# DarlingHang/st-nerf

Hardware: NVIDIA H100
Metric: rays/sec (higher is better)
Workload: dtype f32 via fp16x3 split products (wgmma), f32 accumulate

## Files before the change

### st-nerf_b200/csrc/mlp_tc.cu

```cuda
#include <cuda_fp16.h>
#include <string.h>
#include <type_traits>
#include <vector>
#include "mlp_tc.cuh"
#include "resample.cuh"

namespace stnerf {

namespace {

constexpr int TILE_M = 128;
constexpr int ABLOCK = 16384;
constexpr int STAGE_BYTES = 16384;
constexpr int NTHREADS = 384;
constexpr int MATH_WG0 = 1, N_MATH_WARPS = 8;
constexpr int MAX_STAGE = 8;
constexpr int BAR_WFULL = 0, BAR_WEMPTY = 8, BAR_RAWFULL = 16, BAR_RAWEMPTY = 18;
constexpr int MISC_ROWS = 256;
constexpr int MISC_PART = MISC_ROWS + 128 * 24;
constexpr int MISC_CDF = MISC_PART + 2048;
constexpr int MISC_TOTAL = MISC_CDF + 512;

__device__ __forceinline__ uint32_t smem_u32(const void* p) { return (uint32_t)__cvta_generic_to_shared(p); }

__device__ __forceinline__ void mbar_init(uint32_t bar, uint32_t count) {
  asm volatile("mbarrier.init.shared::cta.b64 [%0], %1;" ::"r"(bar), "r"(count) : "memory");
}
__device__ __forceinline__ void mbar_arrive(uint32_t bar) {
  asm volatile("mbarrier.arrive.shared::cta.b64 _, [%0];" ::"r"(bar) : "memory");
}
__device__ __forceinline__ void mbar_arrive_if(uint32_t bar, bool pred) {
  asm volatile("{\n\t.reg .pred p;\n\tsetp.ne.b32 p, %1, 0;\n\t@p mbarrier.arrive.shared::cta.b64 _, [%0];\n\t}" ::"r"(bar), "r"((uint32_t)pred)
               : "memory");
}
__device__ __forceinline__ void mbar_expect_tx(uint32_t bar, uint32_t bytes) {
  asm volatile("mbarrier.arrive.expect_tx.shared::cta.b64 _, [%0], %1;" ::"r"(bar), "r"(bytes) : "memory");
}
__device__ __forceinline__ void mbar_wait(uint32_t bar, uint32_t parity) {
  asm volatile(
      "{\n\t.reg .pred p;\n\t.reg .u32 c;\n\t"
      "mov.u32 c, 0;\n"
      "WAIT_%=:\n\t"
      "mbarrier.try_wait.parity.shared::cta.b64 p, [%0], %1;\n\t"
      "@p bra.uni DONE_%=;\n\t"
      "add.u32 c, c, 1;\n\t"
      "setp.gt.u32 p, c, 67108864;\n\t"
      "@p trap;\n\t"
      "bra.uni WAIT_%=;\n"
      "DONE_%=:\n\t}" ::"r"(bar), "r"(parity)
      : "memory");
}
__device__ __forceinline__ void bulk_g2s(uint32_t dst, const void* src, uint32_t bytes, uint32_t bar) {
  asm volatile("cp.async.bulk.shared::cluster.global.mbarrier::complete_tx::bytes [%0], [%1], %2, [%3];" ::"r"(dst),
               "l"(src), "r"(bytes), "r"(bar)
               : "memory");
}
__device__ __forceinline__ void fence_proxy_async() { asm volatile("fence.proxy.async.shared::cta;" ::: "memory"); }
__device__ __forceinline__ void wg_bar_sync(int wg) { asm volatile("bar.sync %0, 128;" ::"r"(1 + wg) : "memory"); }

__device__ __forceinline__ void load_stage_elect(uint32_t dst, const void* src, uint32_t bytes, uint32_t bar) {
  asm volatile(
      "{\n\t.reg .pred pe;\n\t"
      "elect.sync _|pe, 0xffffffff;\n\t"
      "@pe mbarrier.arrive.expect_tx.shared::cta.b64 _, [%3], %2;\n\t"
      "@pe cp.async.bulk.shared::cluster.global.mbarrier::complete_tx::bytes [%0], [%1], %2, [%3];\n\t}" ::"r"(dst),
      "l"(src), "r"(bytes), "r"(bar)
      : "memory");
}

__device__ __forceinline__ uint64_t desc_sw128(uint32_t saddr) {
  return (uint64_t)((saddr >> 4) & 0x3FFF) | ((uint64_t)1 << 16) | ((uint64_t)(1024 >> 4) << 32) | ((uint64_t)1 << 62);
}
__device__ __forceinline__ uint64_t desc_sw64(uint32_t saddr) {
  return (uint64_t)((saddr >> 4) & 0x3FFF) | ((uint64_t)1 << 16) | ((uint64_t)(512 >> 4) << 32) | ((uint64_t)2 << 62);
}
__device__ __forceinline__ void wgmma_fence() { asm volatile("wgmma.fence.sync.aligned;" ::: "memory"); }
__device__ __forceinline__ void wgmma_commit() { asm volatile("wgmma.commit_group.sync.aligned;" ::: "memory"); }
template <int N>
__device__ __forceinline__ void wgmma_wait() { asm volatile("wgmma.wait_group.sync.aligned %0;" ::"n"(N) : "memory"); }
template <int R>
__device__ __forceinline__ void acc_fence(float (&d)[128]) {
#pragma unroll
  for (int i = 0; i < R; ++i) asm volatile("" : "+f"(d[i])::"memory");
}

__device__ __forceinline__ void wgmma_n256(float (&d)[128], uint64_t da, uint64_t db) {
  asm volatile(
      "{\n\t.reg .pred p;\n\tsetp.ne.b32 p, %130, 0;\n\t"
      "wgmma.mma_async.sync.aligned.m64n256k16.f32.f16.f16 "
      "{%0, %1, %2, %3, %4, %5, %6, %7, %8, %9, %10, %11, %12, %13, %14, %15, "
      "%16, %17, %18, %19, %20, %21, %22, %23, %24, %25, %26, %27, %28, %29, %30, %31, "
      "%32, %33, %34, %35, %36, %37, %38, %39, %40, %41, %42, %43, %44, %45, %46, %47, "
      "%48, %49, %50, %51, %52, %53, %54, %55, %56, %57, %58, %59, %60, %61, %62, %63, "
      "%64, %65, %66, %67, %68, %69, %70, %71, %72, %73, %74, %75, %76, %77, %78, %79, "
      "%80, %81, %82, %83, %84, %85, %86, %87, %88, %89, %90, %91, %92, %93, %94, %95, "
      "%96, %97, %98, %99, %100, %101, %102, %103, %104, %105, %106, %107, %108, %109, %110, %111, "
      "%112, %113, %114, %115, %116, %117, %118, %119, %120, %121, %122, %123, %124, %125, %126, %127}, "
      "%128, %129, p, 1, 1, 0, 0;\n\t}"
      : "+f"(d[0]), "+f"(d[1]), "+f"(d[2]), "+f"(d[3]), "+f"(d[4]), "+f"(d[5]), "+f"(d[6]), "+f"(d[7]),
        "+f"(d[8]), "+f"(d[9]), "+f"(d[10]), "+f"(d[11]), "+f"(d[12]), "+f"(d[13]), "+f"(d[14]), "+f"(d[15]),
        "+f"(d[16]), "+f"(d[17]), "+f"(d[18]), "+f"(d[19]), "+f"(d[20]), "+f"(d[21]), "+f"(d[22]), "+f"(d[23]),
        "+f"(d[24]), "+f"(d[25]), "+f"(d[26]), "+f"(d[27]), "+f"(d[28]), "+f"(d[29]), "+f"(d[30]), "+f"(d[31]),
        "+f"(d[32]), "+f"(d[33]), "+f"(d[34]), "+f"(d[35]), "+f"(d[36]), "+f"(d[37]), "+f"(d[38]), "+f"(d[39]),
        "+f"(d[40]), "+f"(d[41]), "+f"(d[42]), "+f"(d[43]), "+f"(d[44]), "+f"(d[45]), "+f"(d[46]), "+f"(d[47]),
        "+f"(d[48]), "+f"(d[49]), "+f"(d[50]), "+f"(d[51]), "+f"(d[52]), "+f"(d[53]), "+f"(d[54]), "+f"(d[55]),
        "+f"(d[56]), "+f"(d[57]), "+f"(d[58]), "+f"(d[59]), "+f"(d[60]), "+f"(d[61]), "+f"(d[62]), "+f"(d[63]),
        "+f"(d[64]), "+f"(d[65]), "+f"(d[66]), "+f"(d[67]), "+f"(d[68]), "+f"(d[69]), "+f"(d[70]), "+f"(d[71]),
        "+f"(d[72]), "+f"(d[73]), "+f"(d[74]), "+f"(d[75]), "+f"(d[76]), "+f"(d[77]), "+f"(d[78]), "+f"(d[79]),
        "+f"(d[80]), "+f"(d[81]), "+f"(d[82]), "+f"(d[83]), "+f"(d[84]), "+f"(d[85]), "+f"(d[86]), "+f"(d[87]),
        "+f"(d[88]), "+f"(d[89]), "+f"(d[90]), "+f"(d[91]), "+f"(d[92]), "+f"(d[93]), "+f"(d[94]), "+f"(d[95]),
        "+f"(d[96]), "+f"(d[97]), "+f"(d[98]), "+f"(d[99]), "+f"(d[100]), "+f"(d[101]), "+f"(d[102]), "+f"(d[103]),
        "+f"(d[104]), "+f"(d[105]), "+f"(d[106]), "+f"(d[107]), "+f"(d[108]), "+f"(d[109]), "+f"(d[110]), "+f"(d[111]),
        "+f"(d[112]), "+f"(d[113]), "+f"(d[114]), "+f"(d[115]), "+f"(d[116]), "+f"(d[117]), "+f"(d[118]), "+f"(d[119]),
        "+f"(d[120]), "+f"(d[121]), "+f"(d[122]), "+f"(d[123]), "+f"(d[124]), "+f"(d[125]), "+f"(d[126]), "+f"(d[127])
      : "l"(da), "l"(db), "r"(1));
}
__device__ __forceinline__ void wgmma_n128(float (&d)[128], uint64_t da, uint64_t db) {
  asm volatile(
      "{\n\t.reg .pred p;\n\tsetp.ne.b32 p, %66, 0;\n\t"
      "wgmma.mma_async.sync.aligned.m64n128k16.f32.f16.f16 "
      "{%0, %1, %2, %3, %4, %5, %6, %7, %8, %9, %10, %11, %12, %13, %14, %15, "
      "%16, %17, %18, %19, %20, %21, %22, %23, %24, %25, %26, %27, %28, %29, %30, %31, "
      "%32, %33, %34, %35, %36, %37, %38, %39, %40, %41, %42, %43, %44, %45, %46, %47, "
      "%48, %49, %50, %51, %52, %53, %54, %55, %56, %57, %58, %59, %60, %61, %62, %63}, "
      "%64, %65, p, 1, 1, 0, 0;\n\t}"
      : "+f"(d[0]), "+f"(d[1]), "+f"(d[2]), "+f"(d[3]), "+f"(d[4]), "+f"(d[5]), "+f"(d[6]), "+f"(d[7]),
        "+f"(d[8]), "+f"(d[9]), "+f"(d[10]), "+f"(d[11]), "+f"(d[12]), "+f"(d[13]), "+f"(d[14]), "+f"(d[15]),
        "+f"(d[16]), "+f"(d[17]), "+f"(d[18]), "+f"(d[19]), "+f"(d[20]), "+f"(d[21]), "+f"(d[22]), "+f"(d[23]),
        "+f"(d[24]), "+f"(d[25]), "+f"(d[26]), "+f"(d[27]), "+f"(d[28]), "+f"(d[29]), "+f"(d[30]), "+f"(d[31]),
        "+f"(d[32]), "+f"(d[33]), "+f"(d[34]), "+f"(d[35]), "+f"(d[36]), "+f"(d[37]), "+f"(d[38]), "+f"(d[39]),
        "+f"(d[40]), "+f"(d[41]), "+f"(d[42]), "+f"(d[43]), "+f"(d[44]), "+f"(d[45]), "+f"(d[46]), "+f"(d[47]),
        "+f"(d[48]), "+f"(d[49]), "+f"(d[50]), "+f"(d[51]), "+f"(d[52]), "+f"(d[53]), "+f"(d[54]), "+f"(d[55]),
        "+f"(d[56]), "+f"(d[57]), "+f"(d[58]), "+f"(d[59]), "+f"(d[60]), "+f"(d[61]), "+f"(d[62]), "+f"(d[63])
      : "l"(da), "l"(db), "r"(1));
}

template <int N>
__device__ __forceinline__ void wgmma_k16(float (&d)[128], uint64_t da, uint64_t db) {
  if (N == 256) wgmma_n256(d, da, db);
  else wgmma_n128(d, da, db);
}

__device__ __forceinline__ uint32_t pack_f16x2(float a, float b) {
  uint32_t r;
  asm("cvt.rn.satfinite.f16x2.f32 %0, %1, %2;" : "=r"(r) : "f"(b), "f"(a));
  return r;
}
__device__ __forceinline__ float2 unpack_f16x2(uint32_t p) {
  return __half22float2(*reinterpret_cast<const __half2*>(&p));
}

__host__ __device__ inline uint32_t sw128_offset(int row, int col) {
  return (uint32_t)((row >> 3) * 1024 + (row & 7) * 128 + ((((col >> 3) ^ (row & 7)) & 7) << 4) + ((col & 7) << 1));
}
__host__ __device__ inline uint32_t sw64_offset(int row, int col) {
  return (uint32_t)((row >> 3) * 512 + (row & 7) * 64 + ((((col >> 3) ^ ((row >> 1) & 3)) & 3) << 4) + ((col & 7) << 1));
}

enum { NET_SPACE = 0, NET_MOTION = 1 };

template <int NET> struct Sched;
template <> struct Sched<NET_SPACE> {
  static constexpr int N_LAYERS = 8;
  static constexpr int act_base = 0, enc_base = 8 * ABLOCK;
  static constexpr int LO_STRIDE = 4 * ABLOCK;
  static constexpr int ENC_LO_STRIDE = ABLOCK;
  static constexpr int n_stage = 3, stage_bytes = STAGE_BYTES;
  static constexpr int ring_base = 10 * ABLOCK, misc_base = ring_base + n_stage * stage_bytes, smem_total = misc_base + MISC_TOTAL;
  static_assert(smem_total <= 232448, "shared memory budget (227 KB per CTA)");
  __host__ __device__ static constexpr int n_out(int l) { return l == 7 ? 128 : 256; }
  __host__ __device__ static constexpr int act_chunks(int l) { return l == 0 ? 0 : 4; }
  __host__ __device__ static constexpr int enc_chunks(int l) { return (l == 0 || l == 4) ? 1 : 0; }
  __host__ __device__ static constexpr bool enc_first(int l) { return l == 4; }
};
template <> struct Sched<NET_MOTION> {
  static constexpr int N_LAYERS = 5;
  static constexpr int act_base = 0, enc_base = 0;
  static constexpr int LO_STRIDE = 2 * ABLOCK;
  static constexpr int ENC_LO_STRIDE = 2 * ABLOCK;
  static constexpr int n_stage = 8, stage_bytes = 8192;
  static constexpr int ring_base = 4 * ABLOCK, misc_base = ring_base + n_stage * stage_bytes, smem_total = misc_base + MISC_TOTAL;
  __host__ __device__ static constexpr int n_out(int) { return 128; }
  __host__ __device__ static constexpr int act_chunks(int l) { return l == 0 ? 0 : 2; }
  __host__ __device__ static constexpr int enc_chunks(int l) { return l == 0 ? 2 : 0; }
  __host__ __device__ static constexpr bool enc_first(int) { return false; }
};
static_assert(Sched<NET_SPACE>::n_stage <= MAX_STAGE && Sched<NET_MOTION>::n_stage <= MAX_STAGE, "barrier slots");

enum { A_HI = 0, A_LO = 1, A_HI_LO = 2 };
template <int A>
struct WStep {
  static constexpr int a = A;
  uint32_t offset;
  uint32_t sub;
};
template <int NET>
struct WSched {
  using S = Sched<NET>;
  __host__ __device__ static constexpr int n_chunks(int l) { return S::act_chunks(l) + S::enc_chunks(l); }
  __host__ __device__ static constexpr uint32_t stage_bytes(int l) { return (uint32_t)S::n_out(l) * 64; }
  __host__ __device__ static constexpr size_t layer_bytes(int l) { return (size_t)n_chunks(l) * 2  * 2  * stage_bytes(l); }
  __host__ __device__ static constexpr int chunk_at(int l, int c) {
    return S::enc_first(l) ? (c == 0 ? S::act_chunks(l) : c - 1) : c;
  }
  static constexpr bool enc_first_valid() {
    for (int l = 0; l < S::N_LAYERS; ++l)
      if (S::enc_first(l) && (S::act_chunks(l) == 0 || S::enc_chunks(l) == 0)) return false;
    return true;
  }
  static_assert(enc_first_valid(), "enc_first(l) needs activation chunks and an encoding chunk to reorder");
  template <bool LOFIRST, class C, class F>
  __device__ __forceinline__ static void for_each_step(int l, bool split, C&& chunk, F&& f) {
    const int nact = S::act_chunks(l), nch = nact + S::enc_chunks(l);
    const uint32_t bytes = stage_bytes(l);
    auto at = [&](const auto& a, int c, uint32_t sub, uint32_t lo_stage, auto op) {
      f(a, WStep<decltype(op)::value>{(2 * (2 * (uint32_t)c + sub) + lo_stage) * bytes, sub});
    };
    using HI = std::integral_constant<int, A_HI>;
    using LO = std::integral_constant<int, A_LO>;
    using HI_LO = std::integral_constant<int, A_HI_LO>;
    if (!LOFIRST || !split) {
      for (int c = 0; c < nch; ++c) {
        const auto a = chunk(chunk_at(l, c));
        for (uint32_t sub = 0; sub < 2; ++sub) {
          if (split) { at(a, c, sub, 1u, HI()); at(a, c, sub, 0u, HI_LO()); }
          else at(a, c, sub, 0u, HI());
        }
      }
    } else {
      for (int c = 0; c < nch; ++c) {
        const auto a = chunk(chunk_at(l, c));
        for (uint32_t sub = 0; sub < 2; ++sub) { at(a, c, sub, 1u, HI()); at(a, c, sub, 0u, LO()); }
      }
      for (int c = 0; c < nch; ++c) {
        const auto a = chunk(chunk_at(l, c));
        for (uint32_t sub = 0; sub < 2; ++sub) at(a, c, sub, 0u, HI());
      }
    }
  }
};

template <int NET>
__host__ __device__ constexpr size_t stream_bytes_per_tile() {
  size_t n = 0;
  for (int l = 0; l < Sched<NET>::N_LAYERS; ++l) n += WSched<NET>::layer_bytes(l);
  return n;
}

struct TcParams {
  FuseCoarse fuse;
  PointSrc src;
  const uint8_t* wstream;
  const float* aux;
  const float* cbuf;
  int exact;
  int single_last;
  int lo_first;
  float* raw;
  float* rgb_out;
  float* sigma_out;
  float* xyz_out;
  float* flow_out;
  const int* lerp_flag;
  int lerp_force;
};

constexpr int AUX_BIAS = 0, AUX_WSIG = 8 * 256, AUX_BSIG = AUX_WSIG + 256, AUX_WOUT = AUX_BSIG + 4,
              AUX_BOUT = AUX_WOUT + 3 * 128, AUX_FLOATS = AUX_BOUT + 4;


struct Pt { float x, y, z, tm; int out_index; int cidx; };

__device__ __forceinline__ Pt fetch_pt(const PointSrc& s, long long p, long long n_points) {
  Pt q;
  q.x = q.y = q.z = q.tm = 0.f;
  q.out_index = -1;
  q.cidx = 0;
  if (p >= n_points) return q;
  if (s.mode == SRC_EXPLICIT) {
    const float* pp = s.pos + p * s.pos_stride;
    q.x = pp[0]; q.y = pp[1]; q.z = pp[2];
    if (s.times) q.tm = s.times[p * s.time_stride];
    q.out_index = (int)p;
    q.cidx = (int)p;
    return q;
  }
  const long long slot = p / s.S;
  const int k = (int)(p - slot * s.S);
  const long long ray = s.hit ? (long long)s.hit[slot] : slot;
  const float* rp = s.rays + ray * s.ray_stride;
  q.tm = rp[6 + s.layer];
  q.out_index = (int)(ray * s.S + k);
  q.cidx = (int)slot;
  if (s.mode == SRC_XYZ) {
    q.x = s.pos[3 * p]; q.y = s.pos[3 * p + 1]; q.z = s.pos[3 * p + 2];
    return q;
  }
  if (s.mode == SRC_XYZ_MAP) {
    const int m = s.src_map[ray * s.S + k];
    const float* pp = (m < s.n_first) ? s.pos + 3 * (slot * s.n_first + m) : s.pos2 + 3 * (slot * (s.S - s.n_first) + (m - s.n_first));
    q.x = pp[0]; q.y = pp[1]; q.z = pp[2];
    return q;
  }
  const float tt = s.t[ray * s.S + k];
  float v[3] = {__fadd_rn(__fmul_rn(tt, rp[3]), rp[0]), __fadd_rn(__fmul_rn(tt, rp[4]), rp[1]),
                __fadd_rn(__fmul_rn(tt, rp[5]), rp[2])};
#pragma unroll
  for (int a = 0; a < 3; ++a) {
    if (s.shift_on) v[a] = __fsub_rn(v[a], s.shift[a]);
    if (s.scale_on) v[a] = __fadd_rn(__fdiv_rn(__fsub_rn(v[a], s.pivot[a]), s.scale), s.pivot[a]);
  }
  q.x = v[0]; q.y = v[1]; q.z = v[2];
  return q;
}

struct SinCos3 { float s0, s1, s2, c0, c1, c2; };
struct SinCos4 { float s0, s1, s2, s3, c0, c1, c2, c3; };
__device__ __noinline__ SinCos3 sincos_full3(float x0, float x1, float x2) {
  SinCos3 r;
  sincosf(x0, &r.s0, &r.c0); sincosf(x1, &r.s1, &r.c1); sincosf(x2, &r.s2, &r.c2);
  return r;
}
__device__ __noinline__ SinCos4 sincos_full4(float x0, float x1, float x2, float x3) {
  SinCos4 r;
  sincosf(x0, &r.s0, &r.c0); sincosf(x1, &r.s1, &r.c1); sincosf(x2, &r.s2, &r.c2); sincosf(x3, &r.s3, &r.c3);
  return r;
}

template <int NV>
__device__ __forceinline__ void store_row_split(uint8_t* hi_blk, int lo_stride, int row, int col0, const float (&v)[NV],
                                                bool exact) {
#pragma unroll
  for (int g = 0; g < NV / 8; ++g) {
    uint32_t hp[4], lp[4];
#pragma unroll
    for (int e = 0; e < 4; ++e) {
      const float a = v[g * 8 + 2 * e], b = v[g * 8 + 2 * e + 1];
      hp[e] = pack_f16x2(a, b);
      const float2 hf = unpack_f16x2(hp[e]);
      lp[e] = pack_f16x2(a - hf.x, b - hf.y);
    }
    const uint32_t off = sw128_offset(row, col0 + g * 8);
    *reinterpret_cast<uint4*>(hi_blk + off) = make_uint4(hp[0], hp[1], hp[2], hp[3]);
    if (exact) *reinterpret_cast<uint4*>(hi_blk + lo_stride + off) = make_uint4(lp[0], lp[1], lp[2], lp[3]);
  }
}

template <int half, int piece>
__device__ __forceinline__ void encode_space_piece(uint8_t* smem, const Pt& pt, int row, bool exact, float (&carry)[2]) {
  using S = Sched<NET_SPACE>;
  uint8_t* enc = smem + S::enc_base;
  const float xs[3] = {pt.x, pt.y, pt.z};
  float v[16];
  auto trig = [&](int f, float* dst) {
    const float fr = (float)(1 << f);
    const SinCos3 q = sincos_full3(xs[0] * fr, xs[1] * fr, xs[2] * fr);
    dst[0] = q.s0; dst[1] = q.s1; dst[2] = q.s2; dst[3] = q.c0; dst[4] = q.c1; dst[5] = q.c2;
  };
  if (piece == 0) {
    float t3[6];
    trig(5 * half + 0, v); trig(5 * half + 1, v + 6); trig(5 * half + 2, t3);
    v[12] = t3[0]; v[13] = t3[1]; v[14] = t3[2]; v[15] = t3[3];
    carry[0] = t3[4]; carry[1] = t3[5];
  } else {
    v[0] = carry[0]; v[1] = carry[1];
    trig(5 * half + 3, v + 2); trig(5 * half + 4, v + 8);
    v[14] = half == 0 ? xs[0] : xs[2];
    v[15] = half == 0 ? xs[1] : 0.f;
  }
  store_row_split<16>(enc, S::ENC_LO_STRIDE, row, half * 32 + piece * 16, v, exact);
}

template <int half, int piece>
__device__ __forceinline__ void encode_motion_piece(uint8_t* smem, const Pt& pt, int row, bool exact, bool lerp) {
  using S = Sched<NET_MOTION>;
  uint8_t* enc = smem + S::enc_base + half * ABLOCK;
  const float lo_t = floorf(pt.tm), wgt = pt.tm - lo_t, omw = 1.0f - wgt;
  const float in4[4] = {pt.x, pt.y, pt.z, pt.tm};
  auto trig = [&](int f, float* dst) {
    const float fr = (float)(1 << f);
    if (!lerp) {
      const SinCos4 q = sincos_full4(in4[0] * fr, in4[1] * fr, in4[2] * fr, in4[3] * fr);
      dst[0] = q.s0; dst[1] = q.s1; dst[2] = q.s2; dst[3] = q.s3; dst[4] = q.c0; dst[5] = q.c1; dst[6] = q.c2; dst[7] = q.c3;
    } else {
      const SinCos4 q = sincos_full4(in4[0] * fr, in4[1] * fr, in4[2] * fr, lo_t * fr);
      const SinCos3 q1 = sincos_full3((lo_t + 1.0f) * fr, 0.f, 0.f);
      const float s0[4] = {q.s0, q.s1, q.s2, q.s3}, c0[4] = {q.c0, q.c1, q.c2, q.c3};
      const float s1[4] = {q.s0, q.s1, q.s2, q1.s0}, c1[4] = {q.c0, q.c1, q.c2, q1.c0};
#pragma unroll
      for (int d = 0; d < 4; ++d) {
        dst[d] = __fadd_rn(__fmul_rn(omw, s0[d]), __fmul_rn(wgt, s1[d]));
        dst[4 + d] = __fadd_rn(__fmul_rn(omw, c0[d]), __fmul_rn(wgt, c1[d]));
      }
    }
  };
  float v[16];
  trig(5 * half + 2 * piece, v);
  if (piece < 2) {
    trig(5 * half + 2 * piece + 1, v + 8);
  } else {
#pragma unroll
    for (int d = 0; d < 4; ++d) {
      float a = 0.f;
      if (half == 0) {
        a = in4[d];
        if (lerp) {
          const float lo = d < 3 ? in4[d] : lo_t, hi = d < 3 ? in4[d] : lo_t + 1.0f;
          a = __fadd_rn(__fmul_rn(omw, lo), __fmul_rn(wgt, hi));
        }
      }
      v[8 + d] = a; v[12 + d] = 0.f;
    }
  }
  store_row_split<16>(enc, S::ENC_LO_STRIDE, row, piece * 16, v, exact);
}

template <int NET, int piece>
__device__ __forceinline__ void encode_piece(uint8_t* smem, const Pt& pt, int row, int half, bool exact, bool lerp,
                                             float (&carry)[2]) {
  if (NET == NET_SPACE) {
    if (half == 0) encode_space_piece<0, piece < 2 ? piece : 1>(smem, pt, row, exact, carry);
    else encode_space_piece<1, piece < 2 ? piece : 1>(smem, pt, row, exact, carry);
  } else {
    if (half == 0) encode_motion_piece<0, piece>(smem, pt, row, exact, lerp);
    else encode_motion_piece<1, piece>(smem, pt, row, exact, lerp);
  }
}

template <int NZ>
__device__ __noinline__ void fused_composite_loop(const TcParams& P, const float* rows, float* cdf, uint32_t bar_full, uint32_t bar_empty,
                                                  long long n_tiles, int j, int lane) {
  const FuseCoarse& F = P.fuse;
  const PointSrc& src = P.src;
  const long long n_slots = src.count ? (long long)(*src.count) : src.n_slots;
  const int n1 = 64, n2 = F.n2;
  uint32_t n = 0;
  for (long long tile = blockIdx.x; tile < n_tiles; tile += gridDim.x, ++n) {
    mbar_wait(bar_full, n & 1);
    const long long slot = tile * 2 + j;
    if (slot < n_slots) {
      const long long ray = src.hit ? (long long)src.hit[slot] : slot;
      const float* tp = src.t + ray * n1;
      const float4* rp = reinterpret_cast<const float4*>(rows) + j * 64;
      float t[2], sg[2];
#pragma unroll
      for (int s = 0; s < 2; ++s) {
        const int k = s * 32 + lane;
        const float tk = __ldg(tp + k);
        float v = rp[k].w;
        if (F.is_bkgd) {
          if (tk < F.near_plane) v = 0.0f;
        } else {
          if (tk < 0.0f) v = 0.0f;
          if (F.apply_thr && v < F.thr) v = 0.0f;
        }
        t[s] = tk;
        sg[s] = v;
      }
      const float* up = F.u ? F.u + ray * n2 : nullptr;
      const uint64_t seed = F.seed;
      const uint32_t stream = 64u + (uint32_t)F.layer;
      const unsigned long long gid = F.idmap(F.ray_base + ray);
      rs::LayerOut lo;
      rs::composite_resample_ray<2, NZ>(
          t, sg, n1, n2, F.boarder,
          [rp, lane](int s) {
            const float4 v = rp[s * 32 + lane];
            return make_float3(__fdiv_rn(1.0f, __fadd_rn(1.0f, expf(-v.x))), __fdiv_rn(1.0f, __fadd_rn(1.0f, expf(-v.y))),
                               __fdiv_rn(1.0f, __fadd_rn(1.0f, expf(-v.z))));
          },
          [up, seed, stream, gid](int jj) { return up ? up[jj] : philox_uniform(seed, stream, gid, (uint32_t)jj); },
          cdf, F.t_fine + ray * (n1 + n2), lane, lo, F.z_new ? F.z_new + ray * n2 : nullptr,
          F.z_new ? F.src_map + ray * (n1 + n2) : nullptr);
      if (F.img && lane < 5) {
        const long long rg = F.ray_base + ray;
        const float v = lane == 0 ? lo.pix[0] : lane == 1 ? lo.pix[1] : lane == 2 ? lo.pix[2] : lane == 3 ? lo.pix[3] : lo.pix[4];
        if (F.pixels) F.img[rg * 5 + lane] = v;
        else if (lane < 3) F.img[rg * 3 + lane] = v;
        else F.img[(long long)lane * F.n_total + rg] = v;
      }
    }
    __syncwarp();
    if (lane == 0) mbar_arrive(bar_empty);
  }
}

template <int NET, int N, bool LOFIRST>
__device__ __forceinline__ void mma_layer(float (&acc)[128], int l, bool sp, uint32_t sbase, uint32_t a_row, uint32_t bars,
                                          uint32_t& cnt, int lane) {
  using S = Sched<NET>;
  using W = WSched<NET>;
  constexpr uint32_t NST = S::n_stage;
#pragma unroll
  for (int i = 0; i < N / 2; ++i) acc[i] = 0.f;
  acc_fence<N / 2>(acc);
  wgmma_fence();
  const int nact = S::act_chunks(l);
  int pend = -1;
  auto release = [&](int s) {
    __syncwarp();
    mbar_arrive_if(bars + 8u * (uint32_t)(BAR_WEMPTY + s), lane == 0);
  };
  auto a_block = [&](int ch) {
    uint32_t hi, lo;
    if (ch < nact) {
      hi = sbase + S::act_base + ch * ABLOCK + a_row;
      lo = hi + S::LO_STRIDE;
    } else {
      hi = sbase + S::enc_base + (ch - nact) * ABLOCK + a_row;
      lo = hi + S::ENC_LO_STRIDE;
    }
    return make_uint2(hi, lo);
  };
  W::template for_each_step<LOFIRST>(l, sp, a_block, [&](const uint2& a, auto st) {
    const uint32_t hi = a.x + 64u * st.sub, lo = a.y + 64u * st.sub;
    const uint32_t a0 = decltype(st)::a == A_LO ? lo : hi;
    const uint32_t s = cnt % NST, n = cnt / NST;
    mbar_wait(bars + 8u * (BAR_WFULL + s), n & 1);
    const uint32_t w = sbase + S::ring_base + s * S::stage_bytes;
#pragma unroll
    for (int ks = 0; ks < 2; ++ks) wgmma_k16<N>(acc, desc_sw128(a0 + ks * 32), desc_sw64(w + ks * 32));
    if constexpr (decltype(st)::a == A_HI_LO) {
#pragma unroll
      for (int ks = 0; ks < 2; ++ks) wgmma_k16<N>(acc, desc_sw128(lo + ks * 32), desc_sw64(w + ks * 32));
    }
    wgmma_commit();
    wgmma_wait<1>();
    if (pend >= 0) release(pend);
    pend = (int)s;
    ++cnt;
  });
  wgmma_wait<0>();
  acc_fence<N / 2>(acc);
  release(pend);
}

template <int NET, int N, bool SIGMA>
__device__ __forceinline__ void epi_hidden(const float (&acc)[128], const float* __restrict__ bias, const float* __restrict__ wsig,
                                           uint8_t* smem, int r0, int cq, bool lo_too, float& sig0, float& sig1) {
  using S = Sched<NET>;
#pragma unroll
  for (int j = 0; j < N / 8; ++j) {
    const int col = 8 * j + cq;
    const float2 b = __ldg(reinterpret_cast<const float2*>(bias + col));
    const float v00 = fmaxf(acc[4 * j] + b.x, 0.f), v01 = fmaxf(acc[4 * j + 1] + b.y, 0.f);
    const float v10 = fmaxf(acc[4 * j + 2] + b.x, 0.f), v11 = fmaxf(acc[4 * j + 3] + b.y, 0.f);
    if (SIGMA) {
      const float2 w = __ldg(reinterpret_cast<const float2*>(wsig + col));
      sig0 = fmaf(v00, w.x, sig0); sig0 = fmaf(v01, w.y, sig0);
      sig1 = fmaf(v10, w.x, sig1); sig1 = fmaf(v11, w.y, sig1);
    }
    uint8_t* blk = smem + S::act_base + (col >> 6) * ABLOCK;
    const uint32_t o0 = sw128_offset(r0, col & 63), o1 = sw128_offset(r0 + 8, col & 63);
    const uint32_t h0 = pack_f16x2(v00, v01), h1 = pack_f16x2(v10, v11);
    *reinterpret_cast<uint32_t*>(blk + o0) = h0;
    *reinterpret_cast<uint32_t*>(blk + o1) = h1;
    if (lo_too) {
      const float2 f0 = unpack_f16x2(h0), f1 = unpack_f16x2(h1);
      *reinterpret_cast<uint32_t*>(blk + S::LO_STRIDE + o0) = pack_f16x2(v00 - f0.x, v01 - f0.y);
      *reinterpret_cast<uint32_t*>(blk + S::LO_STRIDE + o1) = pack_f16x2(v10 - f1.x, v11 - f1.y);
    }
  }
}

__device__ __forceinline__ float quad_sum(float v) {
  v += __shfl_xor_sync(0xffffffffu, v, 1);
  v += __shfl_xor_sync(0xffffffffu, v, 2);
  return v;
}

template <int NET, bool LOFIRST>
__global__ void __launch_bounds__(NTHREADS, 1) mlp_tc_kernel(const __grid_constant__ TcParams P) {
  using S = Sched<NET>;
  extern __shared__ __align__(1024) uint8_t smem[];
  const uint32_t sbase = smem_u32(smem);
  if ((sbase & 1023u) != 0) {
    if (threadIdx.x == 0) printf("stnerf mlp_tc: dynamic shared memory base %u is not 1024-byte aligned\n", sbase);
    __trap();
  }
  const uint32_t bars = sbase + S::misc_base;
  auto BAR = [bars](int i) { return bars + 8u * (uint32_t)i; };
  Pt* s_rows = reinterpret_cast<Pt*>(smem + S::misc_base + MISC_ROWS);
  float* s_part = reinterpret_cast<float*>(smem + S::misc_base + MISC_PART);

  const int tid = threadIdx.x, lane = tid & 31;
  const int warp = __shfl_sync(0xffffffffu, tid >> 5, 0);
  const int wgi = __shfl_sync(0xffffffffu, tid >> 7, 0);
  const bool exact = P.exact != 0;
  const bool single_last = P.single_last != 0;
  auto split = [&](int l) { return exact && !(single_last && l == S::N_LAYERS - 1); };
  const long long n_points = src_num_points(P.src);
  const long long n_tiles = (n_points + TILE_M - 1) / TILE_M;
  constexpr uint32_t NST = S::n_stage;
  if (tid == 0) {
    for (int i = 0; i < MAX_STAGE; ++i) { mbar_init(BAR(BAR_WFULL + i), 1); mbar_init(BAR(BAR_WEMPTY + i), N_MATH_WARPS); }
    for (int j = 0; j < 2; ++j) {
      mbar_init(BAR(BAR_RAWFULL + j), 4);
      mbar_init(BAR(BAR_RAWEMPTY + j), 1);
    }
    asm volatile("fence.mbarrier_init.release.cluster;" ::: "memory");
  }
  __syncthreads();

  if (warp == 0) {
    using W = WSched<NET>;
    uint32_t cnt = 0;
    for (long long tile = blockIdx.x; tile < n_tiles; tile += gridDim.x) {
      const uint8_t* layer = P.wstream;
      for (int l = 0; l < S::N_LAYERS; ++l) {
        W::template for_each_step<LOFIRST>(l, split(l), [](int) { return 0; }, [&](int, auto st) {
          const uint32_t s = cnt % NST, n = cnt / NST;
          mbar_wait(BAR(BAR_WEMPTY + s), (n & 1) ^ 1);
          load_stage_elect(sbase + S::ring_base + s * S::stage_bytes, layer + st.offset, W::stage_bytes(l), BAR(BAR_WFULL + s));
          ++cnt;
        });
        layer += W::layer_bytes(l);
      }
    }
  } else if (NET == NET_SPACE && (warp == 2 || warp == 3)) {
    if (P.fuse.on) {
      const int j = warp - 2;
      float* cdf = reinterpret_cast<float*>(smem + S::misc_base + MISC_CDF) + j * 64;
      if (P.fuse.n2 <= 128)
        fused_composite_loop<4>(P, s_part, cdf, BAR(BAR_RAWFULL + j), BAR(BAR_RAWEMPTY + j), n_tiles, j, lane);
      else
        fused_composite_loop<8>(P, s_part, cdf, BAR(BAR_RAWFULL + j), BAR(BAR_RAWEMPTY + j), n_tiles, j, lane);
    }
  } else if (wgi >= MATH_WG0) {
    const int wg = wgi - MATH_WG0;
    const int wt = tid & 127;
    const int erow = wg * 64 + (wt & 63), ehalf = wt >> 6;
    const int r0 = wg * 64 + (wt >> 5) * 16 + (lane >> 2);
    const int cq = 2 * (lane & 3);
    const uint32_t a_row = (uint32_t)wg * 8u * 1024u;
    const float* bias_all = P.aux + AUX_BIAS;
    const bool lerp = (NET == NET_MOTION) && (P.lerp_force >= 0 ? (P.lerp_force != 0) : (P.lerp_flag && *P.lerp_flag != 0));
    const bool fused = (NET == NET_SPACE) && P.fuse.on;
    uint32_t cnt = 0, tile_no = 0;
    float acc[128];
    for (long long tile = blockIdx.x; tile < n_tiles; tile += gridDim.x, ++tile_no) {
      wg_bar_sync(wg);
      const Pt cur = fetch_pt(P.src, tile * TILE_M + erow, n_points);
      if (ehalf == 0) s_rows[erow] = cur;
      float carry[2] = {0.f, 0.f};
      if (NET == NET_MOTION) {
        uint8_t* enc = smem + S::enc_base + ehalf * ABLOCK;
        for (int c = (ehalf == 0 ? 48 : 40); c < 64; c += 8) {
          const uint32_t off = sw128_offset(erow, c);
          *reinterpret_cast<uint4*>(enc + off) = make_uint4(0, 0, 0, 0);
          *reinterpret_cast<uint4*>(enc + S::ENC_LO_STRIDE + off) = make_uint4(0, 0, 0, 0);
        }
      }
      encode_piece<NET, 0>(smem, cur, erow, ehalf, exact, lerp, carry);
      encode_piece<NET, 1>(smem, cur, erow, ehalf, exact, lerp, carry);
      if (NET == NET_MOTION) encode_piece<NET, 2>(smem, cur, erow, ehalf, exact, lerp, carry);
      float sig0 = 0.f, sig1 = 0.f;
      for (int l = 0; l < S::N_LAYERS; ++l) {
        fence_proxy_async();
        wg_bar_sync(wg);
        const bool last = (l == S::N_LAYERS - 1);
        if (!last) {
          mma_layer<NET, (NET == NET_SPACE ? 256 : 128), LOFIRST>(acc, l, split(l), sbase, a_row, bars, cnt, lane);
          if (NET == NET_SPACE && l == 6)
            epi_hidden<NET, 256, true>(acc, bias_all + l * 256, P.aux + AUX_WSIG, smem, r0, cq, split(l + 1), sig0, sig1);
          else
            epi_hidden<NET, (NET == NET_SPACE ? 256 : 128), false>(acc, bias_all + l * 256, nullptr, smem, r0, cq, split(l + 1), sig0, sig1);
          continue;
        }
        mma_layer<NET, 128, LOFIRST>(acc, l, split(l), sbase, a_row, bars, cnt, lane);
        const Pt p0 = s_rows[r0], p1 = s_rows[r0 + 8];
        const float* b0 = (NET == NET_SPACE) ? (P.cbuf + (size_t)p0.cidx * 128) : bias_all + l * 256;
        const float* b1 = (NET == NET_SPACE) ? (P.cbuf + (size_t)p1.cidx * 128) : bias_all + l * 256;
        float d0[3] = {0.f, 0.f, 0.f}, d1[3] = {0.f, 0.f, 0.f};
#pragma unroll
        for (int j = 0; j < 16; ++j) {
          const int col = 8 * j + cq;
          const float2 ba = __ldg(reinterpret_cast<const float2*>(b0 + col));
          const float2 bb = __ldg(reinterpret_cast<const float2*>(b1 + col));
          const float v00 = fmaxf(acc[4 * j] + ba.x, 0.f), v01 = fmaxf(acc[4 * j + 1] + ba.y, 0.f);
          const float v10 = fmaxf(acc[4 * j + 2] + bb.x, 0.f), v11 = fmaxf(acc[4 * j + 3] + bb.y, 0.f);
#pragma unroll
          for (int o = 0; o < 3; ++o) {
            const float2 w = __ldg(reinterpret_cast<const float2*>(P.aux + AUX_WOUT + o * 128 + col));
            d0[o] = fmaf(v00, w.x, d0[o]); d0[o] = fmaf(v01, w.y, d0[o]);
            d1[o] = fmaf(v10, w.x, d1[o]); d1[o] = fmaf(v11, w.y, d1[o]);
          }
        }
#pragma unroll
        for (int o = 0; o < 3; ++o) { d0[o] = quad_sum(d0[o]) + P.aux[AUX_BOUT + o]; d1[o] = quad_sum(d1[o]) + P.aux[AUX_BOUT + o]; }
        if (NET == NET_SPACE) { sig0 = quad_sum(sig0) + P.aux[AUX_BSIG]; sig1 = quad_sum(sig1) + P.aux[AUX_BSIG]; }
        if (fused) {
          if (tile_no > 0) mbar_wait(BAR(BAR_RAWEMPTY + wg), (tile_no - 1) & 1);
          if ((lane & 3) == 0) {
            reinterpret_cast<float4*>(s_part)[r0] = make_float4(d0[0], d0[1], d0[2], sig0);
            reinterpret_cast<float4*>(s_part)[r0 + 8] = make_float4(d1[0], d1[1], d1[2], sig1);
          }
          __syncwarp();
          if (lane == 0) mbar_arrive(BAR(BAR_RAWFULL + wg));
        }
        if ((lane & 3) == 0) {
#pragma unroll
          for (int h = 0; h < 2; ++h) {
            const Pt& p = h ? p1 : p0;
            const float* o = h ? d1 : d0;
            const float sg = h ? sig1 : sig0;
            if (p.out_index < 0) continue;
            const int oi = p.out_index;
            if (NET == NET_SPACE) {
              if (P.raw) reinterpret_cast<float4*>(P.raw)[oi] = make_float4(o[0], o[1], o[2], sg);
              if (P.rgb_out) { P.rgb_out[3 * (size_t)oi] = o[0]; P.rgb_out[3 * (size_t)oi + 1] = o[1]; P.rgb_out[3 * (size_t)oi + 2] = o[2]; }
              if (P.sigma_out) P.sigma_out[oi] = sg;
            } else {
              const long long pidx = tile * TILE_M + r0 + 8 * h;
              if (P.flow_out) { P.flow_out[3 * pidx] = o[0]; P.flow_out[3 * pidx + 1] = o[1]; P.flow_out[3 * pidx + 2] = o[2]; }
              if (P.xyz_out) {
                P.xyz_out[3 * pidx] = __fadd_rn(p.x, o[0]);
                P.xyz_out[3 * pidx + 1] = __fadd_rn(p.y, o[1]);
                P.xyz_out[3 * pidx + 2] = __fadd_rn(p.z, o[2]);
              }
            }
          }
        }
      }
    }
  }
}

constexpr int HB_SLOTS = 8;
__global__ void __launch_bounds__(128) head_bias_kernel(PointSrc src, const float* __restrict__ w_tail ,
                                                        const float* __restrict__ b1, int use_time,
                                                        float* __restrict__ cbuf) {
  __shared__ float s_enc[HB_SLOTS][48];
  const long long n_slots = src.count ? (long long)(*src.count) : src.n_slots;
  const int nk = PE_DIR + (use_time ? PE_TIME : 0);
  const int tid = threadIdx.x;
  float w[48];
#pragma unroll
  for (int k = 0; k < 48; ++k) w[k] = (k < nk) ? __ldg(w_tail + k * 128 + tid) : 0.f;
  const float bias = __ldg(b1 + tid);
  for (long long s0 = (long long)blockIdx.x * HB_SLOTS; s0 < n_slots; s0 += (long long)gridDim.x * HB_SLOTS) {
    __syncthreads();
    for (int e = tid; e < HB_SLOTS * 48; e += 128) {
      const int sl = e / 48, j = e - sl * 48;
      const long long slot = s0 + sl;
      float v = 0.f;
      if (slot < n_slots && j < nk) {
        float d[3], tm;
        if (src.mode == SRC_EXPLICIT) {
          d[0] = src.dirs[3 * slot]; d[1] = src.dirs[3 * slot + 1]; d[2] = src.dirs[3 * slot + 2];
          tm = src.times ? src.times[slot * src.time_stride] : 0.f;
        } else {
          const long long ray = src.hit ? (long long)src.hit[slot] : slot;
          const float* rp = src.rays + ray * src.ray_stride;
          d[0] = rp[3]; d[1] = rp[4]; d[2] = rp[5];
          tm = rp[6 + src.layer];
        }
        if (j < PE_DIR) {
          if (j < 3) v = d[j];
          else {
            const int r = j - 3, f = r / 6, m = r - 6 * f;
            const float a = d[m % 3] * (float)(1 << f);
            v = (m < 3) ? sinf(a) : cosf(a);
          }
        } else {
          const int r = j - PE_DIR;
          if (r == 0) v = tm;
          else {
            const int f = (r - 1) >> 1;
            const float a = tm * (float)(1 << f);
            v = ((r - 1) & 1) ? cosf(a) : sinf(a);
          }
        }
        v = fmaxf(v, 0.f);
      }
      s_enc[sl][j] = v;
    }
    __syncthreads();
#pragma unroll
    for (int sl = 0; sl < HB_SLOTS; ++sl) {
      const long long slot = s0 + sl;
      if (slot >= n_slots) break;
      float acc = bias;
#pragma unroll
      for (int k = 0; k < 48; ++k) acc = fmaf(w[k], s_enc[sl][k], acc);
      cbuf[slot * 128 + tid] = acc;
    }
  }
}

__global__ void __launch_bounds__(256, 1) wgmma_selftest_kernel(const float* __restrict__ A, const uint8_t* __restrict__ Bstages,
                                                               float* __restrict__ D, int reps) {
  extern __shared__ __align__(1024) uint8_t smem[];
  const uint32_t sbase = smem_u32(smem);
  const uint32_t bar = sbase + ABLOCK + 2 * STAGE_BYTES;
  const int tid = threadIdx.x, wg = tid >> 7, wt = tid & 127, lane = tid & 31;
  if ((sbase & 1023u) != 0) __trap();
  if (tid == 0) {
    mbar_init(bar, 1);
    asm volatile("fence.mbarrier_init.release.cluster;" ::: "memory");
  }
  if (tid < 128) {
    for (int c0 = 0; c0 < 64; c0 += 32) {
      float v[32];
      for (int i = 0; i < 32; ++i) v[i] = A[tid * 64 + c0 + i];
      store_row_split<32>(smem, 0, tid, c0, v, false);
    }
  }
  fence_proxy_async();
  __syncthreads();
  if (tid == 0) {
    mbar_expect_tx(bar, 2 * STAGE_BYTES);
    bulk_g2s(sbase + ABLOCK, Bstages, 2 * STAGE_BYTES, bar);
  }
  mbar_wait(bar, 0);
  float acc[128];
#pragma unroll
  for (int i = 0; i < 128; ++i) acc[i] = 0.f;
  acc_fence<128>(acc);
  wgmma_fence();
  for (int rep = 0; rep < reps; ++rep) {
#pragma unroll
    for (int sub = 0; sub < 2; ++sub)
#pragma unroll
      for (int ks = 0; ks < 2; ++ks)
        wgmma_n256(acc, desc_sw128(sbase + (uint32_t)wg * 8192u + sub * 64 + ks * 32),
                   desc_sw64(sbase + ABLOCK + sub * STAGE_BYTES + ks * 32));
    wgmma_commit();
    wgmma_wait<0>();
  }
  acc_fence<128>(acc);
  const int r0 = wg * 64 + (wt >> 5) * 16 + (lane >> 2), cq = 2 * (lane & 3);
#pragma unroll
  for (int j = 0; j < 32; ++j) {
    const int col = 8 * j + cq;
    D[r0 * 256 + col] = acc[4 * j];
    D[r0 * 256 + col + 1] = acc[4 * j + 1];
    D[(r0 + 8) * 256 + col] = acc[4 * j + 2];
    D[(r0 + 8) * 256 + col + 1] = acc[4 * j + 3];
  }
}

struct LayerSpec { const float* W; int N, K_total; std::vector<std::vector<int>> chunks; };

std::vector<int> iota_chunk(int k0, int kend) {
  std::vector<int> c(64, -1);
  for (int i = 0; i < 64 && k0 + i < kend; ++i) c[i] = k0 + i;
  return c;
}
std::vector<int> enc_perm_space(int base) {
  std::vector<int> c(64, -1);
  for (int h = 0; h < 2; ++h) {
    for (int ff = 0; ff < 5; ++ff)
      for (int j = 0; j < 6; ++j) c[h * 32 + 6 * ff + j] = base + 3 + 6 * (5 * h + ff) + j;
    if (h == 0) { c[30] = base + 0; c[31] = base + 1; } else { c[62] = base + 2; }
  }
  return c;
}
std::vector<std::vector<int>> enc_perm_motion() {
  std::vector<std::vector<int>> out(2, std::vector<int>(64, -1));
  for (int h = 0; h < 2; ++h)
    for (int ff = 0; ff < 5; ++ff)
      for (int j = 0; j < 8; ++j) out[h][8 * ff + j] = 4 + 8 * (5 * h + ff) + j;
  for (int d = 0; d < 4; ++d) out[0][40 + d] = d;
  return out;
}

template <int NET>
int pack_stream(TcNet& net, const std::vector<LayerSpec>& layers, const std::vector<float>& aux) {
  std::vector<uint8_t> stream;
  for (int l = 0; l < (int)layers.size(); ++l) {
    const LayerSpec& L = layers[l];
    const size_t stage = (size_t)L.N * 64;
    for (int c = 0; c < (int)L.chunks.size(); ++c) {
      const std::vector<int>& ch = L.chunks[WSched<NET>::chunk_at(l, c)];
      for (int sub = 0; sub < 2; ++sub) {
        std::vector<uint8_t> hi(stage, 0), lo(stage, 0);
        for (int n = 0; n < L.N; ++n)
          for (int c = 0; c < 32; ++c) {
            const int k = ch[sub * 32 + c];
            if (k < 0) continue;
            const float w = L.W[(size_t)n * L.K_total + k];
            const __half h = __float2half_rn(w);
            const __half l = __float2half_rn(w - __half2float(h));
            const uint32_t off = sw64_offset(n, c);
            memcpy(hi.data() + off, &h, 2);
            memcpy(lo.data() + off, &l, 2);
          }
        stream.insert(stream.end(), hi.begin(), hi.end());
        stream.insert(stream.end(), lo.begin(), lo.end());
      }
    }
  }
  if (stream.size() != stream_bytes_per_tile<NET>()) return STNERF_EINVAL;
  tc_free(net);
  net.blob_bytes = stream.size();
  STNERF_CUDA(cudaMalloc(&net.blob, stream.size()));
  STNERF_CUDA(cudaMemcpy(net.blob, stream.data(), stream.size(), cudaMemcpyHostToDevice));
  STNERF_CUDA(cudaMalloc((void**)&net.aux, aux.size() * sizeof(float)));
  STNERF_CUDA(cudaMemcpy(net.aux, aux.data(), aux.size() * sizeof(float), cudaMemcpyHostToDevice));
  return STNERF_OK;
}

}

void tc_free(TcNet& net) {
  if (net.blob) cudaFree(net.blob);
  if (net.aux) cudaFree(net.aux);
  if (net.w_tail) cudaFree(net.w_tail);
  net.blob = nullptr; net.aux = nullptr; net.w_tail = nullptr; net.blob_bytes = 0;
}

size_t tc_stream_bytes(bool is_space) { return is_space ? stream_bytes_per_tile<NET_SPACE>() : stream_bytes_per_tile<NET_MOTION>(); }
size_t tc_aux_floats() { return AUX_FLOATS; }
size_t tc_tail_floats(bool is_space) { return is_space ? 48 * 128 : 0; }

int tc_export(const TcNet& net, bool is_space, uint8_t* stream_host, float* aux_host, float* tail_host) {
  if (!net.blob || !net.aux || net.blob_bytes != tc_stream_bytes(is_space) || (is_space && !net.w_tail)) return STNERF_ENOWEIGHTS;
  STNERF_CUDA(cudaMemcpy(stream_host, net.blob, net.blob_bytes, cudaMemcpyDeviceToHost));
  STNERF_CUDA(cudaMemcpy(aux_host, net.aux, AUX_FLOATS * sizeof(float), cudaMemcpyDeviceToHost));
  if (is_space) STNERF_CUDA(cudaMemcpy(tail_host, net.w_tail, tc_tail_floats(true) * sizeof(float), cudaMemcpyDeviceToHost));
  return STNERF_OK;
}

int tc_import(TcNet& net, bool is_space, int use_time, const uint8_t* stream_host, const float* aux_host, const float* tail_host) {
  tc_free(net);
  net.blob_bytes = tc_stream_bytes(is_space);
  net.use_time = use_time;
  STNERF_CUDA(cudaMalloc(&net.blob, net.blob_bytes));
  STNERF_CUDA(cudaMemcpy(net.blob, stream_host, net.blob_bytes, cudaMemcpyHostToDevice));
  STNERF_CUDA(cudaMalloc((void**)&net.aux, AUX_FLOATS * sizeof(float)));
  STNERF_CUDA(cudaMemcpy(net.aux, aux_host, AUX_FLOATS * sizeof(float), cudaMemcpyHostToDevice));
  if (is_space) {
    STNERF_CUDA(cudaMalloc((void**)&net.w_tail, tc_tail_floats(true) * sizeof(float)));
    STNERF_CUDA(cudaMemcpy(net.w_tail, tail_host, tc_tail_floats(true) * sizeof(float), cudaMemcpyHostToDevice));
  }
  return STNERF_OK;
}

int tc_pack_spacenet(TcNet& net, const float* p, bool use_time) {
  const int krgb = HID + PE_DIR + (use_time ? PE_TIME : 0);
  std::vector<float> aux(AUX_FLOATS, 0.f);
  std::vector<LayerSpec> layers;
  const int Ks[7] = {PE_POS, HID, HID, HID, HID + PE_POS, HID, HID};
  for (int i = 0; i < 7; ++i) {
    LayerSpec L;
    L.W = p; L.N = HID; L.K_total = Ks[i];
    if (i != 0) for (int k = 0; k < HID; k += 64) L.chunks.push_back(iota_chunk(k, HID));
    if (i == 0 || i == 4) L.chunks.push_back(enc_perm_space(i == 0 ? 0 : HID));
    layers.push_back(L);
    p += (size_t)HID * Ks[i];
    memcpy(aux.data() + AUX_BIAS + i * 256, p, HID * sizeof(float));
    p += HID;
  }
  memcpy(aux.data() + AUX_WSIG, p, HID * sizeof(float)); p += HID;
  aux[AUX_BSIG] = *p++;
  LayerSpec L;
  L.W = p; L.N = HEAD; L.K_total = krgb;
  for (int k = 0; k < HID; k += 64) L.chunks.push_back(iota_chunk(k, HID));
  layers.push_back(L);
  std::vector<float> tail(48 * 128, 0.f);
  for (int n = 0; n < HEAD; ++n)
    for (int k = 0; k < krgb - HID; ++k) tail[(size_t)k * 128 + n] = p[(size_t)n * krgb + HID + k];
  p += (size_t)HEAD * krgb;
  memcpy(aux.data() + AUX_BIAS + 7 * 256, p, HEAD * sizeof(float)); p += HEAD;
  memcpy(aux.data() + AUX_WOUT, p, 3 * HEAD * sizeof(float)); p += 3 * HEAD;
  memcpy(aux.data() + AUX_BOUT, p, 3 * sizeof(float));
  net.use_time = use_time ? 1 : 0;
  const int rc = pack_stream<NET_SPACE>(net, layers, aux);
  if (rc) return rc;
  STNERF_CUDA(cudaMalloc((void**)&net.w_tail, tail.size() * sizeof(float)));
  STNERF_CUDA(cudaMemcpy(net.w_tail, tail.data(), tail.size() * sizeof(float), cudaMemcpyHostToDevice));
  return STNERF_OK;
}

int tc_pack_motionnet(TcNet& net, const float* p) {
  std::vector<float> aux(AUX_FLOATS, 0.f);
  std::vector<LayerSpec> layers;
  for (int i = 0; i < 5; ++i) {
    LayerSpec L;
    const int K = i == 0 ? PE_MOTION : HEAD;
    L.W = p; L.N = HEAD; L.K_total = K;
    if (i == 0) L.chunks = enc_perm_motion();
    else for (int k = 0; k < HEAD; k += 64) L.chunks.push_back(iota_chunk(k, HEAD));
    layers.push_back(L);
    p += (size_t)HEAD * K;
    memcpy(aux.data() + AUX_BIAS + i * 256, p, HEAD * sizeof(float));
    p += HEAD;
  }
  memcpy(aux.data() + AUX_WOUT, p, 3 * HEAD * sizeof(float)); p += 3 * HEAD;
  memcpy(aux.data() + AUX_BOUT, p, 3 * sizeof(float));
  return pack_stream<NET_MOTION>(net, layers, aux);
}


int tc_selftest_accum(int reps, float* max_err_host, float* mean_signed_rel_host) {
  if (reps < 1) return STNERF_EINVAL;
  std::vector<float> Af(128 * 64), Bf(256 * 64);
  uint32_t s = 12345u;
  const bool probe = reps > 1;
  auto rnd = [&s, probe]() { s = s * 1664525u + 1013904223u; const float v = ((s >> 8) & 0xFFFF) / 65536.0f; return probe ? 0.5f + 0.5f * v : v - 0.5f; };
  for (auto& v : Af) v = __half2float(__float2half_rn(rnd()));
  for (auto& v : Bf) v = __half2float(__float2half_rn(rnd()));
  std::vector<uint8_t> stages(2 * STAGE_BYTES, 0);
  for (int sub = 0; sub < 2; ++sub)
    for (int n = 0; n < 256; ++n)
      for (int c = 0; c < 32; ++c) {
        const __half h = __float2half_rn(Bf[n * 64 + sub * 32 + c]);
        memcpy(stages.data() + sub * STAGE_BYTES + sw64_offset(n, c), &h, 2);
      }
  float *dA = nullptr, *dD = nullptr; uint8_t* dB = nullptr;
  STNERF_CUDA(cudaMalloc((void**)&dA, Af.size() * 4));
  STNERF_CUDA(cudaMalloc((void**)&dB, stages.size()));
  STNERF_CUDA(cudaMalloc((void**)&dD, 128 * 256 * 4));
  STNERF_CUDA(cudaMemcpy(dA, Af.data(), Af.size() * 4, cudaMemcpyHostToDevice));
  STNERF_CUDA(cudaMemcpy(dB, stages.data(), stages.size(), cudaMemcpyHostToDevice));
  const int smem = ABLOCK + 2 * STAGE_BYTES + 64;
  STNERF_CUDA(cudaFuncSetAttribute(wgmma_selftest_kernel, cudaFuncAttributeMaxDynamicSharedMemorySize, smem));
  wgmma_selftest_kernel<<<1, 256, smem>>>(dA, dB, dD, reps);
  STNERF_LAUNCH_CHECK();
  STNERF_CUDA(cudaDeviceSynchronize());
  std::vector<float> D(128 * 256);
  STNERF_CUDA(cudaMemcpy(D.data(), dD, D.size() * 4, cudaMemcpyDeviceToHost));
  cudaFree(dA); cudaFree(dB); cudaFree(dD);
  float worst = 0.f;
  double signed_rel = 0.0;
  for (int m = 0; m < 128; ++m)
    for (int n = 0; n < 256; ++n) {
      double ref = 0;
      for (int k = 0; k < 64; ++k) ref += (double)Af[m * 64 + k] * Bf[n * 64 + k];
      ref *= reps;
      worst = fmaxf(worst, fabsf((float)(ref - (double)D[m * 256 + n])));
      if (ref != 0.0) signed_rel += ((double)D[m * 256 + n] - ref) / fabs(ref);
    }
  *max_err_host = worst;
  if (mean_signed_rel_host) *mean_signed_rel_host = (float)(signed_rel / (128.0 * 256.0));
  return STNERF_OK;
}
int tc_selftest(float* max_err_host) { return tc_selftest_accum(1, max_err_host, nullptr); }

template <int NET, bool LOFIRST>
static int launch_tc_variant(const TcParams& P, int num_sms, cudaStream_t st) {
  using S = Sched<NET>;
  auto kern = mlp_tc_kernel<NET, LOFIRST>;
  STNERF_CUDA(cudaFuncSetAttribute(kern, cudaFuncAttributeMaxDynamicSharedMemorySize, S::smem_total));
  kern<<<num_sms, NTHREADS, S::smem_total, st>>>(P);
  STNERF_LAUNCH_CHECK();
  return STNERF_OK;
}

template <int NET>
static int launch_tc(const TcParams& P, int num_sms, cudaStream_t st) {
  return P.lo_first ? launch_tc_variant<NET, true>(P, num_sms, st) : launch_tc_variant<NET, false>(P, num_sms, st);
}

bool tc_can_fuse_coarse(int n1, int n2) { return n1 == 64 && n2 >= 1 && n2 <= 256; }

int tc_launch_spacenet(const PointSrc& src, const TcNet& net, int precision, float* cbuf, float* raw,
                       float* rgb_out, float* sigma_out, int num_sms, cudaStream_t st, const FuseCoarse* fuse, bool fine_pass) {
  if (!net.blob || !net.w_tail) return STNERF_ENOWEIGHTS;
  if (!cbuf) return STNERF_EINVAL;
  PointSrc hs = src;
  if (src.mode == SRC_EXPLICIT) hs.count = nullptr;
  const long long slots_hint = src.count ? src.n_slots_cap : src.n_slots;
  long long blocks = (slots_hint + HB_SLOTS - 1) / HB_SLOTS;
  if (blocks < 1) blocks = 1;
  if (blocks > (long long)num_sms * 8) blocks = (long long)num_sms * 8;
  head_bias_kernel<<<(int)blocks, 128, 0, st>>>(hs, net.w_tail, net.aux + AUX_BIAS + 7 * 256, net.use_time, cbuf);
  STNERF_LAUNCH_CHECK();
  TcParams P;
  memset(&P, 0, sizeof(P));
  P.src = src; P.wstream = (const uint8_t*)net.blob; P.aux = net.aux; P.cbuf = cbuf;
  P.exact = precision == STNERF_PREC_TC_3XF16 || precision == STNERF_PREC_TC_MIXED || precision == STNERF_PREC_TC_3XF16_CF;
  P.single_last = precision == STNERF_PREC_TC_MIXED;
  P.raw = raw; P.rgb_out = rgb_out; P.sigma_out = sigma_out; P.lerp_force = 0;
  P.lo_first = precision == STNERF_PREC_TC_3XF16_CF && !fine_pass;
  if (fuse && fuse->on) {
    if (src.mode == SRC_EXPLICIT || src.S != 64 || !tc_can_fuse_coarse(fuse->n1, fuse->n2) || !fuse->t_fine) return STNERF_EINVAL;
    P.fuse = *fuse;
  }
  return launch_tc<NET_SPACE>(P, num_sms, st);
}

int tc_launch_motionnet(const PointSrc& src, const TcNet& net, int precision, const int* lerp_flag_dev,
                        int lerp_force, float* xyz_out, float* flow_out, int num_sms, cudaStream_t st) {
  if (!net.blob) return STNERF_ENOWEIGHTS;
  TcParams P;
  memset(&P, 0, sizeof(P));
  P.src = src; P.wstream = (const uint8_t*)net.blob; P.aux = net.aux;
  P.exact = precision == STNERF_PREC_TC_3XF16 || precision == STNERF_PREC_TC_MIXED || precision == STNERF_PREC_TC_3XF16_CF;
  P.xyz_out = xyz_out; P.flow_out = flow_out; P.lerp_flag = lerp_flag_dev; P.lerp_force = lerp_force;
  P.lo_first = precision == STNERF_PREC_TC_3XF16_CF;
  return launch_tc<NET_MOTION>(P, num_sms, st);
}

}
```

Baseline: 710,000.

## Use stmatrix for epilogue activation stores and scale-d zeroing in wgmma

The hidden-layer epilogue now collects packed fp16 pairs across two column groups and writes them to the 128B-swizzled activation buffer with stmatrix.x4, replacing scattered 32-bit shared stores. This should cut the number of shared-memory store instructions and possible bank conflicts, for both the hi and lo split buffers. Separately, the explicit accumulator zeroing loop is dropped: the first wgmma of each layer now runs with scale_d=0 so it overwrites the accumulator. The swizzle address math for stmatrix must match the wgmma operand layout exactly, or activations will be corrupted.

After: 708,000 (median of 6 runs). About the same (-0.3%).

```diff
diff --git a/st-nerf_b200/csrc/mlp_tc.cu b/st-nerf_b200/csrc/mlp_tc.cu
--- a/st-nerf_b200/csrc/mlp_tc.cu
+++ b/st-nerf_b200/csrc/mlp_tc.cu
@@ -57,6 +57,11 @@
 }
 __device__ __forceinline__ void fence_proxy_async() { asm volatile("fence.proxy.async.shared::cta;" ::: "memory"); }
 __device__ __forceinline__ void wg_bar_sync(int wg) { asm volatile("bar.sync %0, 128;" ::"r"(1 + wg) : "memory"); }
+__device__ __forceinline__ void stmatrix_x4(uint32_t addr, const uint32_t (&r)[4]) {
+  asm volatile("stmatrix.sync.aligned.m8n8.x4.shared.b16 [%0], {%1, %2, %3, %4};" ::"r"(addr), "r"(r[0]), "r"(r[1]), "r"(r[2]),
+               "r"(r[3])
+               : "memory");
+}
 
 __device__ __forceinline__ void load_stage_elect(uint32_t dst, const void* src, uint32_t bytes, uint32_t bar) {
   asm volatile(
@@ -84,7 +89,7 @@
   for (int i = 0; i < R; ++i) asm volatile("" : "+f"(d[i])::"memory");
 }
 
-__device__ __forceinline__ void wgmma_n256(float (&d)[128], uint64_t da, uint64_t db) {
+__device__ __forceinline__ void wgmma_n256(float (&d)[128], uint64_t da, uint64_t db, uint32_t scale_d) {
   asm volatile(
       "{\n\t.reg .pred p;\n\tsetp.ne.b32 p, %130, 0;\n\t"
       "wgmma.mma_async.sync.aligned.m64n256k16.f32.f16.f16 "
@@ -113,9 +118,9 @@
         "+f"(d[104]), "+f"(d[105]), "+f"(d[106]), "+f"(d[107]), "+f"(d[108]), "+f"(d[109]), "+f"(d[110]), "+f"(d[111]),
         "+f"(d[112]), "+f"(d[113]), "+f"(d[114]), "+f"(d[115]), "+f"(d[116]), "+f"(d[117]), "+f"(d[118]), "+f"(d[119]),
         "+f"(d[120]), "+f"(d[121]), "+f"(d[122]), "+f"(d[123]), "+f"(d[124]), "+f"(d[125]), "+f"(d[126]), "+f"(d[127])
-      : "l"(da), "l"(db), "r"(1));
-}
-__device__ __forceinline__ void wgmma_n128(float (&d)[128], uint64_t da, uint64_t db) {
+      : "l"(da), "l"(db), "r"(scale_d));
+}
+__device__ __forceinline__ void wgmma_n128(float (&d)[128], uint64_t da, uint64_t db, uint32_t scale_d) {
   asm volatile(
       "{\n\t.reg .pred p;\n\tsetp.ne.b32 p, %66, 0;\n\t"
       "wgmma.mma_async.sync.aligned.m64n128k16.f32.f16.f16 "
@@ -132,13 +137,13 @@
         "+f"(d[40]), "+f"(d[41]), "+f"(d[42]), "+f"(d[43]), "+f"(d[44]), "+f"(d[45]), "+f"(d[46]), "+f"(d[47]),
         "+f"(d[48]), "+f"(d[49]), "+f"(d[50]), "+f"(d[51]), "+f"(d[52]), "+f"(d[53]), "+f"(d[54]), "+f"(d[55]),
         "+f"(d[56]), "+f"(d[57]), "+f"(d[58]), "+f"(d[59]), "+f"(d[60]), "+f"(d[61]), "+f"(d[62]), "+f"(d[63])
-      : "l"(da), "l"(db), "r"(1));
+      : "l"(da), "l"(db), "r"(scale_d));
 }
 
 template <int N>
-__device__ __forceinline__ void wgmma_k16(float (&d)[128], uint64_t da, uint64_t db) {
-  if (N == 256) wgmma_n256(d, da, db);
-  else wgmma_n128(d, da, db);
+__device__ __forceinline__ void wgmma_k16(float (&d)[128], uint64_t da, uint64_t db, uint32_t scale_d) {
+  if (N == 256) wgmma_n256(d, da, db, scale_d);
+  else wgmma_n128(d, da, db, scale_d);
 }
 
 __device__ __forceinline__ uint32_t pack_f16x2(float a, float b) {
@@ -491,10 +496,8 @@
   using S = Sched<NET>;
   using W = WSched<NET>;
   constexpr uint32_t NST = S::n_stage;
-#pragma unroll
-  for (int i = 0; i < N / 2; ++i) acc[i] = 0.f;
-  acc_fence<N / 2>(acc);
   wgmma_fence();
+  const uint32_t cnt0 = cnt;
   const int nact = S::act_chunks(l);
   int pend = -1;
   auto release = [&](int s) {
@@ -519,10 +522,11 @@
     mbar_wait(bars + 8u * (BAR_WFULL + s), n & 1);
     const uint32_t w = sbase + S::ring_base + s * S::stage_bytes;
 #pragma unroll
-    for (int ks = 0; ks < 2; ++ks) wgmma_k16<N>(acc, desc_sw128(a0 + ks * 32), desc_sw64(w + ks * 32));
+    for (int ks = 0; ks < 2; ++ks)
+      wgmma_k16<N>(acc, desc_sw128(a0 + ks * 32), desc_sw64(w + ks * 32), (ks > 0 || cnt != cnt0) ? 1u : 0u);
     if constexpr (decltype(st)::a == A_HI_LO) {
 #pragma unroll
-      for (int ks = 0; ks < 2; ++ks) wgmma_k16<N>(acc, desc_sw128(lo + ks * 32), desc_sw64(w + ks * 32));
+      for (int ks = 0; ks < 2; ++ks) wgmma_k16<N>(acc, desc_sw128(lo + ks * 32), desc_sw64(w + ks * 32), 1u);
     }
     wgmma_commit();
     wgmma_wait<1>();
@@ -539,6 +543,12 @@
 __device__ __forceinline__ void epi_hidden(const float (&acc)[128], const float* __restrict__ bias, const float* __restrict__ wsig,
                                            uint8_t* smem, int r0, int cq, bool lo_too, float& sig0, float& sig1) {
   using S = Sched<NET>;
+  const int lane = threadIdx.x & 31;
+  const int srow = r0 - (lane >> 2) + ((lane >> 3) & 1) * 8 + (lane & 7);
+  const uint32_t row_off = (uint32_t)((srow >> 3) * 1024 + (srow & 7) * 128);
+  const uint32_t sw = (uint32_t)(((lane >> 4) ^ srow) & 7);
+  const uint32_t base = smem_u32(smem) + S::act_base + row_off;
+  uint32_t hp[4], lp[4];
 #pragma unroll
   for (int j = 0; j < N / 8; ++j) {
     const int col = 8 * j + cq;
@@ -550,15 +560,18 @@
       sig0 = fmaf(v00, w.x, sig0); sig0 = fmaf(v01, w.y, sig0);
       sig1 = fmaf(v10, w.x, sig1); sig1 = fmaf(v11, w.y, sig1);
     }
-    uint8_t* blk = smem + S::act_base + (col >> 6) * ABLOCK;
-    const uint32_t o0 = sw128_offset(r0, col & 63), o1 = sw128_offset(r0 + 8, col & 63);
     const uint32_t h0 = pack_f16x2(v00, v01), h1 = pack_f16x2(v10, v11);
-    *reinterpret_cast<uint32_t*>(blk + o0) = h0;
-    *reinterpret_cast<uint32_t*>(blk + o1) = h1;
+    hp[2 * (j & 1)] = h0;
+    hp[2 * (j & 1) + 1] = h1;
     if (lo_too) {
       const float2 f0 = unpack_f16x2(h0), f1 = unpack_f16x2(h1);
-      *reinterpret_cast<uint32_t*>(blk + S::LO_STRIDE + o0) = pack_f16x2(v00 - f0.x, v01 - f0.y);
-      *reinterpret_cast<uint32_t*>(blk + S::LO_STRIDE + o1) = pack_f16x2(v10 - f1.x, v11 - f1.y);
+      lp[2 * (j & 1)] = pack_f16x2(v00 - f0.x, v01 - f0.y);
+      lp[2 * (j & 1) + 1] = pack_f16x2(v10 - f1.x, v11 - f1.y);
+    }
+    if (j & 1) {
+      const uint32_t a = base + (uint32_t)(j >> 3) * ABLOCK + ((((uint32_t)j & 6u) ^ sw) << 4);
+      stmatrix_x4(a, hp);
+      if (lo_too) stmatrix_x4(a + S::LO_STRIDE, lp);
     }
   }
 }
@@ -824,7 +837,7 @@
 #pragma unroll
       for (int ks = 0; ks < 2; ++ks)
         wgmma_n256(acc, desc_sw128(sbase + (uint32_t)wg * 8192u + sub * 64 + ks * 32),
-                   desc_sw64(sbase + ABLOCK + sub * STAGE_BYTES + ks * 32));
+                   desc_sw64(sbase + ABLOCK + sub * STAGE_BYTES + ks * 32), 1u);
     wgmma_commit();
     wgmma_wait<0>();
   }
```
